# sbarthelemy/arboris-python

Hardware: NVIDIA B200
Metric: world-steps/s (human36, fp64, dt=1ms) (higher is better)
Workload: dtype f64

## Files before the change

arboris-python_b200/csrc/arb_artic.cuh:

```cuda
#pragma once
#include "arb_constraints.cuh"
#include "arb_joints.cuh"
#include "arb_math.cuh"
#include "arb_types.h"

#define FT(ptr, idx) (ptr)[(idx) * ARB_TILE]
#define ST(ptr, idx) (ptr)[(int64_t)(idx) * b.W + w]
ARB_D double arb_ld_state(const double* p) {
#ifdef __CUDA_ARCH__
  double v;
  asm volatile("ld.global.L1::no_allocate.f64 %0, [%1];" : "=d"(v) : "l"(p));
  return v;
#else
  return *p;
#endif
}
#define ST_LD(ptr, idx) arb_ld_state(&ST(ptr, idx))

ARB_HD void wrench_up(const Se3& h, const double* x, double* y) {
  double rm[3], rf[3], c[3];
  m3_mulv(h.R, x, rm);
  m3_mulv(h.R, x + 3, rf);
  cross3(h.p, rf, c);
  y[0] = rm[0] + c[0]; y[1] = rm[1] + c[1]; y[2] = rm[2] + c[2];
// ... 380 lines not shown
#pragma unroll
          for (int i = 0; i < 6; ++i) { IA[6 * r + i] -= U[r] * LA[i]; IM[6 * r + i] -= U[r] * LM[i]; }
          beta[r] += U[r] * u;
        }
      }
    }
    if (par != 0) {
      Se3 X;
      load_se3(b.aX, j, X);
      congruence_up(X, IA);
      congruence_up(X, IM);
      double bu[6];
      wrench_up(X, beta, bu);
      carry = (par == j);
      if (carry) {
#pragma unroll
        for (int i = 0; i < 6; ++i) beta[i] = bu[i];
      } else {
        double* pa = b.aIA + j * (36 * ARB_TILE);
        double* pm = b.aIM + j * (36 * ARB_TILE);
        double* pb = b.abeta + j * (6 * ARB_TILE);
#pragma unroll
        for (int i = 0; i < 36; ++i) { pa[i * ARB_TILE] = IA[i]; pm[i * ARB_TILE] = IM[i]; }
#pragma unroll
        for (int i = 0; i < 6; ++i) pb[i * ARB_TILE] = bu[i];
      }
    } else {
      carry = false;
    }
  }
  return ok;
}

ARB_D bool artic_child_reads_aV(const DevModel& m, int j, int next, bool marked_only) {
  for (int c = m.jchild0[j]; c >= 0; c = m.jsib[c])
    if (c != next && (!marked_only || m.jmark[c])) return true;
  return false;
}
ARB_D bool artic_is_gen_body(const DevModel& m, int j) {
  for (int g = 0; g < m.ngen; ++g)
    if (m.gen_body[g] == j + 1) return true;
  return false;
}
ARB_D int artic_vstride(const DevModel& m) { return 72 * (m.ngen > 1 ? m.ngen : 1); }
ARB_D void artic_down(const Se3& X, double* V, double* Vh) {
  double a[6], c[6];
  iad_apply(X, V, a);
  iad_apply(X, Vh, c);
#pragma unroll
  for (int i = 0; i < 6; ++i) { V[i] = a[i]; Vh[i] = c[i]; }
}

template <bool MARKED_U, int NE, bool PF = true>
ARB_D void artic_forward_full(const DevModel& m, const DevBatch& b, int64_t w, const double* u, double* x,
                              bool ext = false, const int* ek = nullptr) {
  const int n = m.ndof;
  const int VS = artic_vstride(m);
  double V[1 + NE][6], Vh[1 + NE][6];
  int eoff[NE > 0 ? NE : 1], ekc[NE > 0 ? NE : 1];
#pragma unroll
  for (int e = 0; e < NE; ++e) {
    eoff[e] = ext ? m.coloff[m.dofbody[ek[e]]] : 0;
    ekc[e] = ext ? m.dofpos[ek[e]] + 1 : 0;
  }
  int prev = -2;
  for (int j = 0; j < m.nj; ++j) {
    if (PF && j + 1 < m.nj) {
      arb_prefetch_rows<12>(b.aX + (j + 1) * (12 * ARB_TILE));
      artic_prefetch_dofs(m, j + 1, b.aLA, b.aLM, b.aS, b.aSh);
    }
    const int par = m.jparent[j];
    const int nd = arb_joint_ndof(m.jtype[j]);
    const int dof = m.jdof[j];
    const bool ex = NE > 0 && ext && m.jmark[j];
    if (par == 0) {
#pragma unroll
      for (int r = 0; r < 1 + NE; ++r)
#pragma unroll
        for (int i = 0; i < 6; ++i) { V[r][i] = 0.; Vh[r][i] = 0.; }
    } else {
      Se3 X;
      load_se3(b.aX, j, X);
      const bool reload = (par - 1 != prev);
      if (reload) {
#pragma unroll
        for (int i = 0; i < 6; ++i) { V[0][i] = FT(b.aV, (par - 1) * VS + i); Vh[0][i] = FT(b.aV, (par - 1) * VS + 6 + i); }
      }
      artic_down(X, V[0], Vh[0]);
      if (ex) {
#pragma unroll
        for (int e = 1; e < 1 + NE; ++e) {
          if (reload) {
#pragma unroll
            for (int i = 0; i < 6; ++i) {
              V[e][i] = FT(b.aV, (par - 1) * VS + e * 12 + i);
              Vh[e][i] = FT(b.aV, (par - 1) * VS + e * 12 + 6 + i);
            }
          }
          artic_down(X, V[e], Vh[e]);
        }
      }
    }
    const bool useu = !MARKED_U || m.jmark[j];
    for (int c = 0; c < nd; ++c) {
      const int k = dof + c;
      double LA[6], LM[6], s[6], sh[6];
#pragma unroll
      for (int i = 0; i < 6; ++i) {
        LA[i] = FT(b.aLA, k * 6 + i); LM[i] = FT(b.aLM, k * 6 + i);
        s[i] = FT(b.aS, k * 6 + i); sh[i] = FT(b.aSh, k * 6 + i);
      }
      double t = useu ? FT(u, k) : 0.;
      if (par != 0 || c > 0) {
#pragma unroll
        for (int i = 0; i < 6; ++i) t -= LA[i] * V[0][i] + LM[i] * Vh[0][i];
      }
      FT(x, k) = t;
#pragma unroll
      for (int i = 0; i < 6; ++i) { V[0][i] += s[i] * t; Vh[0][i] += sh[i] * t; }
      if (ex) {
        const int pos = m.dofpos[k];
#pragma unroll
        for (int e = 0; e < NE; ++e) {
          const bool onpath = pos < ekc[e] && m.pathdof[eoff[e] + pos] == k;
          double te = onpath ? FT(b.au, (1 + e) * n + k) : 0.;
          if (par != 0 || c > 0) {
#pragma unroll
            for (int i = 0; i < 6; ++i) te -= LA[i] * V[1 + e][i] + LM[i] * Vh[1 + e][i];
          }
          FT(b.ax, e * n + k) = te;
#pragma unroll
          for (int i = 0; i < 6; ++i) { V[1 + e][i] += s[i] * te; Vh[1 + e][i] += sh[i] * te; }
        }
      }
    }
    const bool gen = !MARKED_U && m.jmark[j] && artic_is_gen_body(m, j);
    if (gen || artic_child_reads_aV(m, j, j + 1, false)) {
#pragma unroll
      for (int i = 0; i < 6; ++i) { FT(b.aV, j * VS + i) = V[0][i]; FT(b.aV, j * VS + 6 + i) = Vh[0][i]; }
    }
    if (ex && (gen || artic_child_reads_aV(m, j, j + 1, true))) {
#pragma unroll
      for (int e = 1; e < 1 + NE; ++e)
#pragma unroll
        for (int i = 0; i < 6; ++i) { FT(b.aV, j * VS + e * 12 + i) = V[e][i]; FT(b.aV, j * VS + e * 12 + 6 + i) = Vh[e][i]; }
    }
    prev = j;
  }
}

template <int NR>
ARB_D void artic_backward_generators(const DevModel& m, const DevBatch& b, int64_t w, int body, int kstart,
                                     const double* rot = nullptr, int ubase = 0) {
  const int n = m.ndof;
  const int off = m.coloff[body];
  double beta[NR][6];
#pragma unroll
  for (int r = 0; r < NR; ++r)
#pragma unroll
    for (int i = 0; i < 6; ++i) beta[r][i] = (kstart < 0 && i == r) ? -1. : 0.;
  if (rot != nullptr && NR == 6) {
#pragma unroll
    for (int r = 0; r < NR; ++r)
#pragma unroll
      for (int i = 0; i < 6; ++i) beta[r][i] = ((r < 3) == (i < 3)) ? -rot[3 * (r % 3) + (i % 3)] : 0.;
  }
  const int l0 = (kstart < 0) ? m.kcols[body] - 1 : m.dofpos[kstart];
  for (int l = l0; l >= 0; --l) {
    const int k = m.pathdof[off + l];
    const int j = m.dofjoint[k];
    if (l > 0) {
      const int kn = m.pathdof[off + l - 1];
      arb_prefetch_rows<6>(b.aS + kn * (6 * ARB_TILE));
      arb_prefetch_rows<6>(b.aU + kn * (6 * ARB_TILE));
      arb_prefetch(b.adinv + kn * ARB_TILE);
    }
    double s[6], U[6];
#pragma unroll
    for (int i = 0; i < 6; ++i) { s[i] = FT(b.aS, k * 6 + i); U[i] = FT(b.aU, k * 6 + i); }
    const double dinv = FT(b.adinv, k);
    const bool last = (l == 0);
#pragma unroll
    for (int r = 0; r < NR; ++r) {
      double sb = 0.;
#pragma unroll
      for (int i = 0; i < 6; ++i) sb += s[i] * beta[r][i];
      const double tau = (k == kstart) ? 1. : 0.;
      const double u = (tau - sb) * dinv;
      FT(b.au, (ubase + r) * n + k) = u;
      if (!last) {
#pragma unroll
        for (int i = 0; i < 6; ++i) beta[r][i] += U[i] * u;
      }
    }
    if (k == m.jdof[j] && m.jparent[j] != 0) {
      Se3 X;
      load_se3(b.aX, j, X);
#pragma unroll
      for (int r = 0; r < NR; ++r) {
        double y[6];
        wrench_up(X, beta[r], y);
#pragma unroll
        for (int i = 0; i < 6; ++i) beta[r][i] = y[i];
      }
    }
  }
}

template <int NR, bool CARRY>
ARB_D void artic_forward_generators(const DevModel& m, const DevBatch& b, int64_t w, int body, int kstart) {
  const int n = m.ndof;
  const int VS = artic_vstride(m);
  const int off = m.coloff[body];
  const int kc = ((kstart < 0) ? m.kcols[body] - 1 : m.dofpos[kstart]) + 1;
  double V[NR][6], Vh[NR][6];
  int prev = -2;
  for (int j = 0; j < m.nj; ++j) {
    if (!m.jmark[j]) continue;
    int jn = j + 1;
    while (jn < m.nj && !m.jmark[jn]) ++jn;
    if (jn < m.nj) {
      arb_prefetch_rows<12>(b.aX + jn * (12 * ARB_TILE));
      artic_prefetch_dofs(m, jn, b.aLA, b.aLM, b.aS, b.aSh);
    }
    const int par = m.jparent[j];
    const int nd = arb_joint_ndof(m.jtype[j]);
    const int dof = m.jdof[j];
    if (par == 0) {
#pragma unroll
      for (int r = 0; r < NR; ++r)
#pragma unroll
        for (int i = 0; i < 6; ++i) { V[r][i] = 0.; Vh[r][i] = 0.; }
    } else {
      Se3 X;
      load_se3(b.aX, j, X);
      const bool reload = !CARRY || (par - 1 != prev);
#pragma unroll
      for (int r = 0; r < NR; ++r) {
        if (reload) {
#pragma unroll
          for (int i = 0; i < 6; ++i) {
            V[r][i] = FT(b.aV, (par - 1) * VS + r * 12 + i);
            Vh[r][i] = FT(b.aV, (par - 1) * VS + r * 12 + 6 + i);
          }
        }
        artic_down(X, V[r], Vh[r]);
      }
    }
    for (int c = 0; c < nd; ++c) {
      const int k = dof + c;
      const int pos = m.dofpos[k];
      const bool onpath = pos < kc && m.pathdof[off + pos] == k;
      double LA[6], LM[6], s[6], sh[6];
#pragma unroll
      for (int i = 0; i < 6; ++i) {
        LA[i] = FT(b.aLA, k * 6 + i); LM[i] = FT(b.aLM, k * 6 + i);
        s[i] = FT(b.aS, k * 6 + i); sh[i] = FT(b.aSh, k * 6 + i);
      }
#pragma unroll
      for (int r = 0; r < NR; ++r) {
        double t = onpath ? FT(b.au, r * n + k) : 0.;
        if (par != 0 || c > 0) {
#pragma unroll
          for (int i = 0; i < 6; ++i) t -= LA[i] * V[r][i] + LM[i] * Vh[r][i];
        }
        FT(b.ax, r * n + k) = t;
#pragma unroll
        for (int i = 0; i < 6; ++i) { V[r][i] += s[i] * t; Vh[r][i] += sh[i] * t; }
      }
    }
    if (!CARRY || artic_child_reads_aV(m, j, jn, true)) {
#pragma unroll
      for (int r = 0; r < NR; ++r)
#pragma unroll
        for (int i = 0; i < 6; ++i) {
          FT(b.aV, j * VS + r * 12 + i) = V[r][i];
          FT(b.aV, j * VS + r * 12 + 6 + i) = Vh[r][i];
        }
    } else if (artic_is_gen_body(m, j)) {
#pragma unroll
      for (int r = 0; r < NR; ++r)
#pragma unroll
        for (int i = 0; i < 6; ++i) FT(b.aV, j * VS + r * 12 + i) = V[r][i];
    }
    prev = j;
  }
}

ARB_D void artic_forward_generators_all(const DevModel& m, const DevBatch& b, int64_t w) {
  const int n = m.ndof;
  const int VS = artic_vstride(m);
  for (int j = 0; j < m.nj; ++j) {
    if (!m.jmark[j]) continue;
    int jn = j + 1;
    while (jn < m.nj && !m.jmark[jn]) ++jn;
    if (jn < m.nj) {
      arb_prefetch_rows<12>(b.aX + jn * (12 * ARB_TILE));
      artic_prefetch_dofs(m, jn, b.aLA, b.aLM, b.aS, b.aSh);
    }
    const int par = m.jparent[j];
    const int nd = arb_joint_ndof(m.jtype[j]);
    const int dof = m.jdof[j];
    for (int gi = 0; gi < m.ngen; ++gi) {
      const int off = m.coloff[m.gen_body[gi]];
      const int kc = m.kcols[m.gen_body[gi]];
      const int rb = 6 * gi;
      double V[6][6], Vh[6][6];
      if (par == 0) {
#pragma unroll
        for (int r = 0; r < 6; ++r)
#pragma unroll
          for (int i = 0; i < 6; ++i) { V[r][i] = 0.; Vh[r][i] = 0.; }
      } else {
        Se3 X;
        load_se3(b.aX, j, X);
#pragma unroll
        for (int r = 0; r < 6; ++r) {
#pragma unroll
          for (int i = 0; i < 6; ++i) {
            V[r][i] = FT(b.aV, (par - 1) * VS + (rb + r) * 12 + i);
            Vh[r][i] = FT(b.aV, (par - 1) * VS + (rb + r) * 12 + 6 + i);
          }
          artic_down(X, V[r], Vh[r]);
        }
        if (m.jmarkfirst[j]) {
          const bool pgen = artic_is_gen_body(m, par - 1);
#pragma unroll
          for (int r = 0; r < 6; ++r) {
            const double* pv = b.aV + ((par - 1) * VS + (rb + r) * 12) * ARB_TILE;
            if (!pgen) arb_discard_rows<6>(pv);
            arb_discard_rows<6>(pv + 6 * ARB_TILE);
          }
        }
      }
      for (int c = 0; c < nd; ++c) {
        const int k = dof + c;
        const int pos = m.dofpos[k];
        const bool onpath = pos < kc && m.pathdof[off + pos] == k;
        double LA[6], LM[6], s[6], sh[6];
#pragma unroll
        for (int i = 0; i < 6; ++i) {
          LA[i] = FT(b.aLA, k * 6 + i); LM[i] = FT(b.aLM, k * 6 + i);
          s[i] = FT(b.aS, k * 6 + i); sh[i] = FT(b.aSh, k * 6 + i);
        }
#pragma unroll
        for (int r = 0; r < 6; ++r) {
          double t = onpath ? FT(b.au, (rb + r) * n + k) : 0.;
          if (par != 0 || c > 0) {
#pragma unroll
            for (int i = 0; i < 6; ++i) t -= LA[i] * V[r][i] + LM[i] * Vh[r][i];
          }
          if (m.doflim[k]) FT(b.ax, (rb + r) * n + k) = t;
#pragma unroll
          for (int i = 0; i < 6; ++i) { V[r][i] += s[i] * t; Vh[r][i] += sh[i] * t; }
        }
      }
      const bool vh_read = m.jmarkchild[j] != 0;
#pragma unroll
      for (int r = 0; r < 6; ++r)
#pragma unroll
        for (int i = 0; i < 6; ++i) {
          FT(b.aV, j * VS + (rb + r) * 12 + i) = V[r][i];
          if (vh_read) FT(b.aV, j * VS + (rb + r) * 12 + 6 + i) = Vh[r][i];
        }
    }
  }
}

#ifndef ARTIC_GEN_CARRY
#define ARTIC_GEN_CARRY 0
#endif
template <int NR>
ARB_D void artic_solve_generators(const DevModel& m, const DevBatch& b, int64_t w, int body, int kstart,
                                  const double* rot = nullptr) {
  artic_backward_generators<NR>(m, b, w, body, kstart, rot, 0);
  artic_forward_generators<NR, (ARTIC_GEN_CARRY != 0)>(m, b, w, body, kstart);
}

ARB_D double artic_gen_value(const DevModel& m, const DevBatch& b, int64_t w, int g, int r, const double* x) {
  if (g < 6 * m.ngen) return FT(b.aV, (m.gen_body[g / 6] - 1) * artic_vstride(m) + r * 12 + g % 6);
  return FT(x, r * m.ndof + m.glimdof[g - 6 * m.ngen]);
}
ARB_D void artic_gen_block(const DevModel& m, const DevBatch& b, int gi, int r, const double* rot, double* out) {
  double V[6];
#pragma unroll
  for (int i = 0; i < 6; ++i) V[i] = FT(b.aV, (m.gen_body[gi] - 1) * artic_vstride(m) + r * 12 + i);
  if (rot != nullptr) {
    m3_mulv(rot, V, out);
    m3_mulv(rot, V + 3, out + 3);
  } else {
#pragma unroll
    for (int i = 0; i < 6; ++i) out[i] = V[i];
  }
}

ARB_D void artic_backward_wrenches(const DevModel& m, const DevBatch& b, int64_t w, const double* y) {
  const int NG6 = 6 * m.ngen;
  for (int j = m.nj - 1; j >= 0; --j) {
    if (!m.jmark[j]) continue;
    const int par = m.jparent[j];
    const int nd = arb_joint_ndof(m.jtype[j]);
    const int dof = m.jdof[j];
    double beta[6] = {0., 0., 0., 0., 0., 0.};
    for (int g = 0; g < m.ngen; ++g)
      if (m.gen_body[g] == j + 1) {
        if (m.gen_aligned[g]) {
          double Re[9], yy[6], t[6];
#pragma unroll
          for (int i = 0; i < 9; ++i) Re[i] = FT(b.fRe, 9 * g + i);
#pragma unroll
          for (int i = 0; i < 6; ++i) yy[i] = FT(y, 6 * g + i);
          m3t_mulv(Re, yy, t);
          m3t_mulv(Re, yy + 3, t + 3);
#pragma unroll
          for (int i = 0; i < 6; ++i) beta[i] -= t[i];
        } else {
#pragma unroll
          for (int i = 0; i < 6; ++i) beta[i] -= FT(y, 6 * g + i);
        }
// ... 32 lines not shown
```

arboris-python_b200/csrc/arb_fused.cuh:

```cuda
#pragma once
#include "arb_artic.cuh"
#include "arb_constraints.cuh"
#include "arb_world.cuh"

ARB_D DevBatch fused_tile_view(const DevBatch& b, int64_t w) {
  DevBatch t = b;
  const int64_t tile = w / ARB_TILE, lane = w % ARB_TILE;
  const int64_t od = tile * b.frec * ARB_TILE + lane, oi = tile * b.firec * ARB_TILE + lane;
  t.fq += od; t.fLam += od; t.fv0 += od; t.fT1 += od; t.fT0 += od; t.fu += od; t.fy += od;
  t.fAcc += od; t.fP += od; t.faux += od; t.fpose += od; t.ff += od; t.fRe += od;
  t.aX += od; t.atw += od; t.ath += od; t.aS += od; t.aSh += od; t.aU += od; t.aLA += od;
  t.aLM += od; t.adinv += od; t.aIA += od; t.aIM += od; t.abeta += od; t.au += od; t.ax += od;
  t.aV += od; t.fK += od;
  t.factive += oi; t.fbranch += oi; t.fzidx += oi;
  return t;
}

ARB_D bool constraint_update(const DevModel& m, int c, const Se3& P0, const Se3& P1, const double* TW0,
                             const double* TW1, double q, double dt, double* aux, double* T1,
                             double* T0, int* zidx, bool aligned = false) {
  const int type = m.ctype[c];
  const double* cd = m.cdbl + ARB_CONS_NDBL * c;
  if (type == ARB_CONS_JOINT_LIMITS) {
    aux[0] = q;
// ... 28 lines not shown
    aux[0] = sdist;
    r0 = 2; nr = 4;
    if (!active) return false;
    if (aligned) {
      const double d[3] = {P1.p[0] - Hc0.p[0], P1.p[1] - Hc0.p[1], P1.p[2] - Hc0.p[2]};
      m3t_mulv(Hc0.R, d, T1);
      return true;
    }
  }
  Se3 F0, F1, F0i, H01;
  se3_mul(P0, cb0, F0);
  se3_mul(P1, cb1, F1);
  se3_inv(F0, F0i);
  se3_mul(F0i, F1, H01);
  if (type == ARB_CONS_BALL_SOCKET) {
#pragma unroll
    for (int i = 0; i < 3; ++i) aux[i] = H01.p[i];
  }
#pragma unroll
  for (int col = 0; col < 6; ++col) {
    double e[6] = {0., 0., 0., 0., 0., 0.}, y[6], z[6];
    e[col] = 1.;
    iad_apply(cb1, e, y);
    ad_apply(H01, y, z);
    for (int r = 0; r < nr; ++r) T1[r * 6 + col] = z[r0 + r];
    iad_apply(cb0, e, y);
    for (int r = 0; r < nr; ++r) T0[r * 6 + col] = y[r0 + r];
  }
  return true;
}

template <int NR>
ARB_D void fused_gen_rows(const DevModel& m, const DevBatch& b, int64_t w, const double* x, double* out,
                          int stride, int col0, int rv0 = 0) {
  for (int gj = 0; gj < m.ngen; ++gj) {
    double Re[9];
    const bool al = m.gen_aligned[gj] != 0;
    if (al) {
#pragma unroll
      for (int i = 0; i < 9; ++i) Re[i] = FT(b.fRe, 9 * gj + i);
    }
#pragma unroll
    for (int r = 0; r < NR; ++r) {
      double v[6];
      artic_gen_block(m, b, gj, rv0 + r, al ? Re : nullptr, v);
#pragma unroll
      for (int i = 0; i < 6; ++i) FT(out, (6 * gj + i) * stride + col0 + r) = v[i];
    }
  }
  for (int g = 6 * m.ngen; g < m.ngrows; ++g)
#pragma unroll
    for (int r = 0; r < NR; ++r) FT(out, g * stride + col0 + r) = FT(x, r * m.ndof + m.glimdof[g - 6 * m.ngen]);
}

template <bool APPLIED = false>
ARB_D void world_fused_prepare(const DevModel& m, const DevBatch& b, int64_t w, double dt,
                               const DevApplied& ap = DevApplied{nullptr, nullptr, nullptr}) {
  const int NG = m.ngrows;
  artic_kinematics(m, b, w);
  if (!artic_factor<APPLIED>(m, b, w, dt, ap)) b.status[w] |= ARB_STATUS_SINGULAR;
  for (int gi = 0; gi < m.ngen; ++gi) {
    if (!m.gen_aligned[gi]) continue;
    double Rc[9], Rb[9], Re[9];
    int zi[3];
    zaligned(m.cdbl + ARB_CONS_NDBL * m.gen_c0[gi] + 32, Rc, zi);
#pragma unroll
    for (int i = 0; i < 9; ++i) Rb[i] = FT(b.fpose, (m.gen_body[gi] - 1) * 12 + i);
#pragma unroll
    for (int i = 0; i < 3; ++i)
#pragma unroll
      for (int j = 0; j < 3; ++j) Re[3 * i + j] = Rc[i] * Rb[j] + Rc[3 + i] * Rb[3 + j] + Rc[6 + i] * Rb[6 + j];
#pragma unroll
    for (int i = 0; i < 9; ++i) FT(b.fRe, 9 * gi + i) = Re[i];
  }
  bool any = false;
  for (int c = 0; c < m.nc; ++c) {
    const int* ci = m.cint + ARB_CONS_NINT * c;
    const int type = m.ctype[c];
// ... 12 lines not shown
    } else {
      Se3 P0, P1;
      double TW0[6], TW1[6];
      if (ci[0] == 0) se3_identity(P0); else load_se3(b.fpose, ci[0] - 1, P0);
      if (ci[1] == 0) se3_identity(P1); else load_se3(b.fpose, ci[1] - 1, P1);
#pragma unroll
      for (int i = 0; i < 6; ++i) {
        TW0[i] = (ci[0] == 0) ? 0. : FT(b.atw, (ci[0] - 1) * 6 + i);
        TW1[i] = (ci[1] == 0) ? 0. : FT(b.atw, (ci[1] - 1) * 6 + i);
      }
      const bool aligned = m.caligned[c] != 0;
      act = constraint_update(m, c, P0, P1, TW0, TW1, 0., dt, aux, T1, T0, zi, aligned);
      if (type == ARB_CONS_SOFT_FINGER_PLANE_POINT) {
#pragma unroll
        for (int i = 0; i < 4; ++i) ST(b.cforce, r0 + i) = 0.;
#pragma unroll
        for (int i = 0; i < 3; ++i) FT(b.fzidx, 3 * c + i) = zi[i];
      }
      if (act) {
        if (aligned) {
#pragma unroll
          for (int i = 0; i < 3; ++i) FT(b.fT1, c * 24 + i) = T1[i];
        } else {
          const int nr = arb_cons_ndol(type);
          for (int i = 0; i < nr * 6; ++i) { FT(b.fT1, c * 24 + i) = T1[i]; FT(b.fT0, c * 24 + i) = T0[i]; }
        }
      }
    }
#pragma unroll
    for (int i = 0; i < 4; ++i) FT(b.faux, 4 * c + i) = aux[i];
    FT(b.factive, c) = act ? 1 : 0;
    any = any || act;
  }
  const int nlim = NG - 6 * m.ngen;
  const int nm = nlim >= 2 ? 2 : 0;
  if (nm == 2) {
    const int ek[2] = {m.glimdof[0], m.glimdof[1]};
    if (any) {
      artic_backward_generators<1>(m, b, w, m.dofbody[ek[0]], ek[0], nullptr, 1);
      artic_backward_generators<1>(m, b, w, m.dofbody[ek[1]], ek[1], nullptr, 2);
    }
    artic_forward_full<false, 2>(m, b, w, b.au, b.fq, any, ek);
  } else {
    artic_forward_full<false, 0>(m, b, w, b.au, b.fq);
  }
  if (!any) return;
  fused_gen_rows<1>(m, b, w, b.fq, b.fv0, 1, 0);
  for (int e = 0; e < nm; ++e)
    fused_gen_rows<1>(m, b, w, b.ax + e * m.ndof * ARB_TILE, b.fLam, NG, 6 * m.ngen + e, 1 + e);
#ifndef PREP_GEN_SEPARATE
  for (int gi = 0; gi < m.ngen; ++gi) {
    if (m.gen_aligned[gi]) {
      double Re[9];
#pragma unroll
      for (int i = 0; i < 9; ++i) Re[i] = FT(b.fRe, 9 * gi + i);
      artic_backward_generators<6>(m, b, w, m.gen_body[gi], -1, Re, 6 * gi);
    } else {
      artic_backward_generators<6>(m, b, w, m.gen_body[gi], -1, nullptr, 6 * gi);
    }
  }
  artic_forward_generators_all(m, b, w);
  for (int gi = 0; gi < m.ngen; ++gi)
    fused_gen_rows<6>(m, b, w, b.ax + 6 * gi * m.ndof * ARB_TILE, b.fLam, NG, 6 * gi, 6 * gi);
#else
  for (int gi = 0; gi < m.ngen; ++gi) {
    if (m.gen_aligned[gi]) {
      double Re[9];
#pragma unroll
      for (int i = 0; i < 9; ++i) Re[i] = FT(b.fRe, 9 * gi + i);
      artic_solve_generators<6>(m, b, w, m.gen_body[gi], -1, Re);
    } else {
      artic_solve_generators<6>(m, b, w, m.gen_body[gi], -1);
    }
    fused_gen_rows<6>(m, b, w, b.ax, b.fLam, NG, 6 * gi);
  }
#endif
  for (int h = 6 * m.ngen + nm; h < NG; ++h) {
    const int k = m.glimdof[h - 6 * m.ngen];
    artic_solve_generators<1>(m, b, w, m.dofbody[k], k);
    fused_gen_rows<1>(m, b, w, b.ax, b.fLam, NG, h);
  }
}

#ifdef __CUDA_ARCH__
#define arb_warp_any(pred) (__any_sync(__activemask(), (pred)) != 0)
#else
#define arb_warp_any(pred) (pred)
#endif

ARB_D void gs_prefetch_visit(const DevModel& m, const DevBatch& b, int c) {
  const int r0 = m.crow[c];
  const double* Tp = ((m.cgen1[c] < 0) ? b.fT0 : b.fT1) + c * (24 * ARB_TILE);
  const double* pA = b.fAcc + r0 * (4 * ARB_TILE);
  const double* pP = b.fP + r0 * (4 * ARB_TILE);
  if (m.caligned[c]) {
#pragma unroll
    for (int i = 0; i < 3; ++i) arb_prefetch(Tp + i * ARB_TILE);
  } else {
#pragma unroll
    for (int i = 0; i < 24; ++i) arb_prefetch(Tp + i * ARB_TILE);
  }
#pragma unroll
  for (int i = 0; i < 16; ++i) { arb_prefetch(pA + i * ARB_TILE); arb_prefetch(pP + i * ARB_TILE); }
}

struct GsCache {
  int g, n;
  double u[6], dy[6];
  double* L;
  int ls;
};
#define GSL(k, i) (k).L[(i) * (k).ls]

ARB_D void gs_cache_flush(const DevModel& m, const DevBatch& b, int64_t w, GsCache& k) {
// ... 1200 lines not shown
      if (needs && k.g != gF) {
        gs_cache_flush(m, b, w, k);
        gs_cache_load<true>(m, b, w, k, gF, 6);
      }
      if (type == ARB_CONS_BALL_SOCKET) {
        if (act) gs_visit_one_body<3>(m, b, w, c, dt, k, &status);
        continue;
      }
      double f[4], df[4];
      int br = 0, slot = 0;
      if (act) {
        if (c + 1 < m.nc) gs_prefetch_visit(m, b, c + 1);
        br = gs_softfinger_begin(m, b, c, dt, k, co, f, df, &slot, &status);
      }
      coop_solve_sliding(co, m.cdbl + ARB_CONS_NDBL * c + 37);
      if (act) gs_softfinger_end(m, b, c, k, co, br, slot, f, df, &status);
      if (br == 3 && c < 32) slid |= 1u << c;
    }
  }
  if (live) {
    gs_cache_flush(m, b, w, k);
    gs_final_wrench(m, b);
    for (int r = 0; r < m.nrows; ++r) ST(b.cforce, r) = FT(b.ff, r);
    if (status) b.status[w] |= status;
  }
  return gs_sort_key(m, slid, (unsigned)(amask & 0xffffffffull));
}

ARB_D void world_fused_finish(const DevModel& m, const DevBatch& b, int64_t w, double dt) {
  bool any = false;
  for (int c = 0; c < m.nc; ++c) any = any || FT(b.factive, c);
  if (any) {
    artic_backward_wrenches(m, b, w, b.fy);
    artic_forward_full<true, 0, false>(m, b, w, b.au, b.ax);
  }
  bool finite = true;
  for (int j = 0; j < m.nj; ++j) {
    const int type = m.jtype[j];
    const int g = m.jgpos[j], d = m.jdof[j];
    const int nd = arb_joint_ndof(type);
    double nv[6];
    for (int i = 0; i < nd; ++i) {
      double t = FT(b.fq, d + i);
      if (any) t += FT(b.ax, d + i);
      ST(b.gvel, d + i) = t;
      finite = finite && isfinite(t);
      nv[i] = t;
    }
    if (type == ARB_JOINT_FREE) {
      double q[16], tw[6];
      for (int i = 0; i < 16; ++i) q[i] = ST_LD(b.gpos, g + i);
#pragma unroll
      for (int i = 0; i < 6; ++i) tw[i] = dt * nv[i];
      Se3 H, E, R;
      se3_from16(q, H);
      se3_exp(tw, E);
      se3_mul(H, E, R);
#pragma unroll
      for (int r = 0; r < 3; ++r) {
#pragma unroll
        for (int c = 0; c < 3; ++c) ST(b.gpos, g + 4 * r + c) = R.R[3 * r + c];
        ST(b.gpos, g + 4 * r + 3) = R.p[r];
      }
    } else {
      for (int i = 0; i < nd; ++i) ST(b.gpos, g + i) = ST_LD(b.gpos, g + i) + dt * nv[i];
    }
  }
// ... 3 lines not shown
```

arboris-python_b200/csrc/arb_model_host.h:

```cpp
#pragma once
#include <cmath>
#include <cstring>
#include <string>
#include <vector>
#include "arb_math.cuh"
#include "arb_types.h"

struct HostModel {
  int ndof = 0, ngpos = 0, nj = 0, nc = 0, na = 0, nrows = 0, ncols = 0, maxk = 0, anyvisc = 0;
  std::vector<int> jtype, jparent, jdof, jgpos, hcn_ident, bflags, coloff, kcols, pathdof;
  std::vector<int> ctype, cint, crow, atype, aint;
  std::vector<int> dofbody, dofpos, gen_body, cgen1, cgen0;
  std::vector<int> gen_aligned, gen_c0, caligned;
  std::vector<int> doflim;
  std::vector<unsigned> crunmask;
  int ngen = 0, ngrows = 0;
  std::vector<int> dofjoint, jhaschild, jaccfirst, jmark, jmarkfirst, jmarkchild, glimdof, pd_gpos;
  std::vector<int> pd_index, pd_dofs;
  int has_warm = 0;
  std::vector<int> glev_off, glev_joint, gslot, gvslot;
  GroupLayout gl;
  std::vector<int> jchild0, jsib;
  std::vector<double> pd_kp, pd_kd, pd_qd, pd_c, pd_dqd;
  int has_pd = 0, nweight = 0;
// ... 315 lines not shown
  }
  int64_t total_ints() const { return cactive + cbranch + cdol + czidx; }
};
static inline ScratchSizes scratch_sizes(const HostModel& m) {
  ScratchSizes s;
  const int64_t n = m.ndof, nj = m.nj, nr = m.nrows > 0 ? m.nrows : 1, nc = m.nc > 0 ? m.nc : 1;
  s.pose = nj * 12; s.twist = nj * 6; s.J = (int64_t)m.ncols * 6; s.dJ = s.J;
  s.M = s.N = s.B = s.Z = s.Y = n * n; s.gforce = n;
  s.cjac = nr * n; s.cvel = nr; s.cA = nr * nr; s.cT = n * nr; s.cpinv = nr * 4; s.caux = nc * 4;
  s.tmp = 2 * n;
  s.cactive = s.cbranch = s.cdol = nc; s.czidx = nc * 3;
  return s;
}
struct FusedSizes {
  int64_t fq, fLam, fv0, fT1, fT0, fu, fy, fAcc, fP, faux, fpose, ff, fRe, factive, fbranch, fzidx;
  int64_t aX, atw, ath, aS, aSh, aU, aLA, aLM, adinv, aIA, aIM, abeta, au, ax, aV, fK;
  int64_t total_doubles() const {
    return fq + fLam + fv0 + fT1 + fT0 + fu + fy + fAcc + fP + faux + fpose + ff + fRe +
           aX + atw + ath + aS + aSh + aU + aLA + aLM + adinv + aIA + aIM + abeta + au + ax + aV + fK;
  }
  int64_t total_ints() const { return factive + fbranch + fzidx; }
};
static inline FusedSizes fused_sizes(const HostModel& m) {
  FusedSizes s;
  const int64_t n = m.ndof, NG = m.ngrows > 0 ? m.ngrows : 1, nc = m.nc > 0 ? m.nc : 1,
                nr = m.nrows > 0 ? m.nrows : 1;
  const int64_t nj = m.nj > 0 ? m.nj : 1, nn = n > 0 ? n : 1;
  s.fq = nn; s.fLam = NG * NG; s.fv0 = NG; s.fT1 = nc * 24; s.fT0 = nc * 24;
  s.fu = NG; s.fy = NG; s.fAcc = nr * 4; s.fP = nr * 4; s.faux = nc * 4; s.fpose = nj * 12; s.ff = nr;
  s.fRe = 9 * (m.ngen > 0 ? m.ngen : 1);
  s.factive = nc; s.fbranch = nc; s.fzidx = 3 * nc;
  s.aX = nj * 12; s.atw = nj * 6; s.ath = nj * 6;
  s.aS = s.aSh = s.aU = s.aLA = s.aLM = nn * 6; s.adinv = nn;
  s.aIA = s.aIM = nj * 36; s.abeta = nj * 6;
  const int64_t ng1 = m.ngen > 1 ? m.ngen : 1;
  s.au = 6 * ng1 * nn; s.ax = 6 * ng1 * nn; s.aV = nj * 72 * ng1;
  s.fK = nn * NG;
  return s;
}
static inline int64_t fused_padded_worlds(int64_t W) { return (W + ARB_TILE - 1) / ARB_TILE * ARB_TILE; }
static inline void carve_fused(const FusedSizes& s, double* dbl, int* ints, DevBatch& b) {
  double* p = dbl;
  auto take = [&](int64_t k) { double* r = p; p += k * ARB_TILE; return r; };
  b.fq = take(s.fq); b.fLam = take(s.fLam); b.fv0 = take(s.fv0);
  b.fT1 = take(s.fT1); b.fT0 = take(s.fT0); b.fu = take(s.fu); b.fy = take(s.fy);
  b.fAcc = take(s.fAcc); b.fP = take(s.fP); b.faux = take(s.faux); b.fpose = take(s.fpose);
  b.ff = take(s.ff); b.fRe = take(s.fRe);
  b.aX = take(s.aX); b.atw = take(s.atw); b.ath = take(s.ath);
  b.aS = take(s.aS); b.aSh = take(s.aSh); b.aU = take(s.aU); b.aLA = take(s.aLA); b.aLM = take(s.aLM);
  b.adinv = take(s.adinv); b.aIA = take(s.aIA); b.aIM = take(s.aIM); b.abeta = take(s.abeta);
  b.au = take(s.au); b.ax = take(s.ax); b.aV = take(s.aV);
  b.fK = take(s.fK);
  int* q = ints;
  auto takei = [&](int64_t k) { int* r = q; q += k * ARB_TILE; return r; };
  b.factive = takei(s.factive); b.fbranch = takei(s.fbranch); b.fzidx = takei(s.fzidx);
  b.frec = s.total_doubles();
  b.firec = s.total_ints();
}
static inline int applied_wrench_rows(const HostModel& m, int nbodies, const int32_t* bodies, bool has_wrench,
                                      std::vector<int>& rows, std::string& err) {
  if (nbodies < 0) { err = "negative number of wrench bodies"; return -1; }
  if (nbodies > 0 && !bodies) { err = "null body list"; return -1; }
  if (has_wrench && nbodies == 0) { err = "a wrench array needs its bodies"; return -1; }
  rows.assign(m.nj > 0 ? m.nj : 1, -1);
  for (int i = 0; i < nbodies; ++i) {
    const int body = bodies[i];
    if (body == 0) { err = "no wrench can be applied to the ground (body 0)"; return -1; }
    if (body < 0 || body > m.nj) { err = "wrench body " + std::to_string(body) + " out of range"; return -1; }
    if (rows[body - 1] >= 0) { err = "wrench body " + std::to_string(body) + " listed twice"; return -1; }
// ... 18 lines not shown
```

Before: 23.54 million.

## Fuse all generator backward/forward sweeps into single per-joint tree passes

Replaces the separate backward and forward articulated-body sweeps, previously run once per generator group (6-row body generators and single-row joint-limit rows), with one backward pass over marked joints that handles every group per joint. Generator columns are also folded into the main forward_full sweep per joint. Partial beta wrenches are carried across joints in an abeta slot buffer, and the aV/au/ax buffers are resized to hold all NG rows. The aim is fewer traversals of the tree and reuse of per-joint S/U/LA/LM loads across groups, at the cost of larger per-world scratch buffers and more global memory traffic for the carried state.

After: 21.86 million, median of 6. 0.929x the previous value.

```diff
diff --git a/arboris-python_b200/csrc/arb_artic.cuh b/arboris-python_b200/csrc/arb_artic.cuh
--- a/arboris-python_b200/csrc/arb_artic.cuh
+++ b/arboris-python_b200/csrc/arb_artic.cuh
@@ -436,6 +436,16 @@
   return ok;
 }
 
+ARB_D int artic_vstride(const DevModel& m) { return 12 * (1 + m.ngrows); }
+
+#ifdef ARB_HOSTTEST_COUNTERS
+#define ARB_ROWREADS_MAXJ 256
+static long arb_rowreads[2][ARB_ROWREADS_MAXJ];
+#define ARB_COUNT_ROWS(dir, j) do { if ((j) < ARB_ROWREADS_MAXJ) ++arb_rowreads[dir][j]; } while (0)
+#else
+#define ARB_COUNT_ROWS(dir, j) do { } while (0)
+#endif
+
 ARB_D bool artic_child_reads_aV(const DevModel& m, int j, int next, bool marked_only) {
   for (int c = m.jchild0[j]; c >= 0; c = m.jsib[c])
     if (c != next && (!marked_only || m.jmark[c])) return true;
@@ -446,7 +456,6 @@
     if (m.gen_body[g] == j + 1) return true;
   return false;
 }
-ARB_D int artic_vstride(const DevModel& m) { return 72 * (m.ngen > 1 ? m.ngen : 1); }
 ARB_D void artic_down(const Se3& X, double* V, double* Vh) {
   double a[6], c[6];
   iad_apply(X, V, a);
@@ -455,20 +464,83 @@
   for (int i = 0; i < 6; ++i) { V[i] = a[i]; Vh[i] = c[i]; }
 }
 
-template <bool MARKED_U, int NE, bool PF = true>
-ARB_D void artic_forward_full(const DevModel& m, const DevBatch& b, int64_t w, const double* u, double* x,
-                              bool ext = false, const int* ek = nullptr) {
+template <int NR>
+ARB_D void artic_forward_group(const DevModel& m, const DevBatch& b, int j, int g0, int off, int kc) {
   const int n = m.ndof;
   const int VS = artic_vstride(m);
-  double V[1 + NE][6], Vh[1 + NE][6];
-  int eoff[NE > 0 ? NE : 1], ekc[NE > 0 ? NE : 1];
-#pragma unroll
-  for (int e = 0; e < NE; ++e) {
-    eoff[e] = ext ? m.coloff[m.dofbody[ek[e]]] : 0;
-    ekc[e] = ext ? m.dofpos[ek[e]] + 1 : 0;
-  }
+  const int cv = 1 + g0;
+  const int par = m.jparent[j];
+  const int nd = arb_joint_ndof(m.jtype[j]);
+  const int dof = m.jdof[j];
+  double V[NR][6], Vh[NR][6];
+  if (par == 0) {
+#pragma unroll
+    for (int r = 0; r < NR; ++r)
+#pragma unroll
+      for (int i = 0; i < 6; ++i) { V[r][i] = 0.; Vh[r][i] = 0.; }
+  } else {
+    Se3 X;
+    load_se3(b.aX, j, X);
+#pragma unroll
+    for (int r = 0; r < NR; ++r) {
+#pragma unroll
+      for (int i = 0; i < 6; ++i) {
+        V[r][i] = FT(b.aV, (par - 1) * VS + (cv + r) * 12 + i);
+        Vh[r][i] = FT(b.aV, (par - 1) * VS + (cv + r) * 12 + 6 + i);
+      }
+      artic_down(X, V[r], Vh[r]);
+    }
+    if (m.jmarkfirst[j]) {
+      const bool pgen = artic_is_gen_body(m, par - 1);
+#pragma unroll
+      for (int r = 0; r < NR; ++r) {
+        const double* pv = b.aV + ((par - 1) * VS + (cv + r) * 12) * ARB_TILE;
+        if (!pgen) arb_discard_rows<6>(pv);
+        arb_discard_rows<6>(pv + 6 * ARB_TILE);
+      }
+    }
+  }
+  for (int c = 0; c < nd; ++c) {
+    const int k = dof + c;
+    const int pos = m.dofpos[k];
+    const bool onpath = pos < kc && m.pathdof[off + pos] == k;
+    double LA[6], LM[6], s[6], sh[6];
+#pragma unroll
+    for (int i = 0; i < 6; ++i) {
+      LA[i] = FT(b.aLA, k * 6 + i); LM[i] = FT(b.aLM, k * 6 + i);
+      s[i] = FT(b.aS, k * 6 + i); sh[i] = FT(b.aSh, k * 6 + i);
+    }
+#pragma unroll
+    for (int r = 0; r < NR; ++r) {
+      double t = onpath ? FT(b.au, (cv + r) * n + k) : 0.;
+      if (par != 0 || c > 0) {
+#pragma unroll
+        for (int i = 0; i < 6; ++i) t -= LA[i] * V[r][i] + LM[i] * Vh[r][i];
+      }
+      if (m.doflim[k]) FT(b.ax, (g0 + r) * n + k) = t;
+#pragma unroll
+      for (int i = 0; i < 6; ++i) { V[r][i] += s[i] * t; Vh[r][i] += sh[i] * t; }
+    }
+  }
+  const bool vh_read = m.jmarkchild[j] != 0;
+#pragma unroll
+  for (int r = 0; r < NR; ++r)
+#pragma unroll
+    for (int i = 0; i < 6; ++i) {
+      FT(b.aV, j * VS + (cv + r) * 12 + i) = V[r][i];
+      if (vh_read) FT(b.aV, j * VS + (cv + r) * 12 + 6 + i) = Vh[r][i];
+    }
+}
+
+template <bool MARKED_U, bool GEN, bool PF = true>
+ARB_D void artic_forward_full(const DevModel& m, const DevBatch& b, int64_t w, const double* u, double* x,
+                              bool gens = false) {
+  const int VS = artic_vstride(m);
+  const int NG6 = 6 * m.ngen;
+  double V[6], Vh[6];
   int prev = -2;
   for (int j = 0; j < m.nj; ++j) {
+    ARB_COUNT_ROWS(1, j);
     if (PF && j + 1 < m.nj) {
       arb_prefetch_rows<12>(b.aX + (j + 1) * (12 * ARB_TILE));
       artic_prefetch_dofs(m, j + 1, b.aLA, b.aLM, b.aS, b.aSh);
@@ -476,34 +548,17 @@
     const int par = m.jparent[j];
     const int nd = arb_joint_ndof(m.jtype[j]);
     const int dof = m.jdof[j];
-    const bool ex = NE > 0 && ext && m.jmark[j];
     if (par == 0) {
 #pragma unroll
-      for (int r = 0; r < 1 + NE; ++r)
-#pragma unroll
-        for (int i = 0; i < 6; ++i) { V[r][i] = 0.; Vh[r][i] = 0.; }
+      for (int i = 0; i < 6; ++i) { V[i] = 0.; Vh[i] = 0.; }
     } else {
       Se3 X;
       load_se3(b.aX, j, X);
-      const bool reload = (par - 1 != prev);
-      if (reload) {
-#pragma unroll
-        for (int i = 0; i < 6; ++i) { V[0][i] = FT(b.aV, (par - 1) * VS + i); Vh[0][i] = FT(b.aV, (par - 1) * VS + 6 + i); }
-      }
-      artic_down(X, V[0], Vh[0]);
-      if (ex) {
-#pragma unroll
-        for (int e = 1; e < 1 + NE; ++e) {
-          if (reload) {
-#pragma unroll
-            for (int i = 0; i < 6; ++i) {
-              V[e][i] = FT(b.aV, (par - 1) * VS + e * 12 + i);
-              Vh[e][i] = FT(b.aV, (par - 1) * VS + e * 12 + 6 + i);
-            }
-          }
-          artic_down(X, V[e], Vh[e]);
-        }
-      }
+      if (par - 1 != prev) {
+#pragma unroll
+        for (int i = 0; i < 6; ++i) { V[i] = FT(b.aV, (par - 1) * VS + i); Vh[i] = FT(b.aV, (par - 1) * VS + 6 + i); }
+      }
+      artic_down(X, V, Vh);
     }
     const bool useu = !MARKED_U || m.jmark[j];
     for (int c = 0; c < nd; ++c) {
@@ -517,68 +572,60 @@
       double t = useu ? FT(u, k) : 0.;
       if (par != 0 || c > 0) {
 #pragma unroll
-        for (int i = 0; i < 6; ++i) t -= LA[i] * V[0][i] + LM[i] * Vh[0][i];
+        for (int i = 0; i < 6; ++i) t -= LA[i] * V[i] + LM[i] * Vh[i];
       }
       FT(x, k) = t;
 #pragma unroll
-      for (int i = 0; i < 6; ++i) { V[0][i] += s[i] * t; Vh[0][i] += sh[i] * t; }
-      if (ex) {
-        const int pos = m.dofpos[k];
-#pragma unroll
-        for (int e = 0; e < NE; ++e) {
-          const bool onpath = pos < ekc[e] && m.pathdof[eoff[e] + pos] == k;
-          double te = onpath ? FT(b.au, (1 + e) * n + k) : 0.;
-          if (par != 0 || c > 0) {
-#pragma unroll
-            for (int i = 0; i < 6; ++i) te -= LA[i] * V[1 + e][i] + LM[i] * Vh[1 + e][i];
-          }
-          FT(b.ax, e * n + k) = te;
-#pragma unroll
-          for (int i = 0; i < 6; ++i) { V[1 + e][i] += s[i] * te; Vh[1 + e][i] += sh[i] * te; }
-        }
-      }
+      for (int i = 0; i < 6; ++i) { V[i] += s[i] * t; Vh[i] += sh[i] * t; }
     }
     const bool gen = !MARKED_U && m.jmark[j] && artic_is_gen_body(m, j);
     if (gen || artic_child_reads_aV(m, j, j + 1, false)) {
 #pragma unroll
-      for (int i = 0; i < 6; ++i) { FT(b.aV, j * VS + i) = V[0][i]; FT(b.aV, j * VS + 6 + i) = Vh[0][i]; }
-    }
-    if (ex && (gen || artic_child_reads_aV(m, j, j + 1, true))) {
-#pragma unroll
-      for (int e = 1; e < 1 + NE; ++e)
-#pragma unroll
-        for (int i = 0; i < 6; ++i) { FT(b.aV, j * VS + e * 12 + i) = V[e][i]; FT(b.aV, j * VS + e * 12 + 6 + i) = Vh[e][i]; }
+      for (int i = 0; i < 6; ++i) { FT(b.aV, j * VS + i) = V[i]; FT(b.aV, j * VS + 6 + i) = Vh[i]; }
     }
     prev = j;
+    if (GEN && gens && m.jmark[j]) {
+      for (int gi = 0; gi < m.ngen; ++gi)
+        artic_forward_group<6>(m, b, j, 6 * gi, m.coloff[m.gen_body[gi]], m.kcols[m.gen_body[gi]]);
+      for (int g = NG6; g < m.ngrows; ++g) {
+        const int k = m.glimdof[g - NG6];
+        artic_forward_group<1>(m, b, j, g, m.coloff[m.dofbody[k]], m.dofpos[k] + 1);
+      }
+    }
   }
 }
 
 template <int NR>
-ARB_D void artic_backward_generators(const DevModel& m, const DevBatch& b, int64_t w, int body, int kstart,
-                                     const double* rot = nullptr, int ubase = 0) {
+ARB_D void artic_backward_group(const DevModel& m, const DevBatch& b, int j, int g0, int body, int kstart, int rot) {
   const int n = m.ndof;
-  const int off = m.coloff[body];
+  const int dof = m.jdof[j];
+  const int p0 = m.dofpos[dof];
+  const int l0 = (kstart < 0) ? m.kcols[body] - 1 : m.dofpos[kstart];
+  if (p0 > l0 || m.pathdof[m.coloff[body] + p0] != dof) return;
+  double* slot = b.abeta + g0 * (6 * ARB_TILE);
   double beta[NR][6];
-#pragma unroll
-  for (int r = 0; r < NR; ++r)
-#pragma unroll
-    for (int i = 0; i < 6; ++i) beta[r][i] = (kstart < 0 && i == r) ? -1. : 0.;
-  if (rot != nullptr && NR == 6) {
+  if (j == body - 1) {
 #pragma unroll
     for (int r = 0; r < NR; ++r)
 #pragma unroll
-      for (int i = 0; i < 6; ++i) beta[r][i] = ((r < 3) == (i < 3)) ? -rot[3 * (r % 3) + (i % 3)] : 0.;
-  }
-  const int l0 = (kstart < 0) ? m.kcols[body] - 1 : m.dofpos[kstart];
-  for (int l = l0; l >= 0; --l) {
-    const int k = m.pathdof[off + l];
-    const int j = m.dofjoint[k];
-    if (l > 0) {
-      const int kn = m.pathdof[off + l - 1];
-      arb_prefetch_rows<6>(b.aS + kn * (6 * ARB_TILE));
-      arb_prefetch_rows<6>(b.aU + kn * (6 * ARB_TILE));
-      arb_prefetch(b.adinv + kn * ARB_TILE);
-    }
+      for (int i = 0; i < 6; ++i) beta[r][i] = (kstart < 0 && i == r) ? -1. : 0.;
+    if (rot >= 0 && NR == 6) {
+      const double* R = b.fRe + 9 * rot * ARB_TILE;
+#pragma unroll
+      for (int r = 0; r < NR; ++r)
+#pragma unroll
+        for (int i = 0; i < 6; ++i) beta[r][i] = ((r < 3) == (i < 3)) ? -FT(R, 3 * (r % 3) + (i % 3)) : 0.;
+    }
+  } else {
+#pragma unroll
+    for (int r = 0; r < NR; ++r)
+#pragma unroll
+      for (int i = 0; i < 6; ++i) beta[r][i] = FT(slot, 6 * r + i);
+  }
+  for (int c = arb_joint_ndof(m.jtype[j]) - 1; c >= 0; --c) {
+    const int l = p0 + c;
+    if (l > l0) continue;
+    const int k = dof + c;
     double s[6], U[6];
 #pragma unroll
     for (int i = 0; i < 6; ++i) { s[i] = FT(b.aS, k * 6 + i); U[i] = FT(b.aU, k * 6 + i); }
@@ -591,204 +638,58 @@
       for (int i = 0; i < 6; ++i) sb += s[i] * beta[r][i];
       const double tau = (k == kstart) ? 1. : 0.;
       const double u = (tau - sb) * dinv;
-      FT(b.au, (ubase + r) * n + k) = u;
+      FT(b.au, (1 + g0 + r) * n + k) = u;
       if (!last) {
 #pragma unroll
         for (int i = 0; i < 6; ++i) beta[r][i] += U[i] * u;
       }
     }
-    if (k == m.jdof[j] && m.jparent[j] != 0) {
-      Se3 X;
-      load_se3(b.aX, j, X);
-#pragma unroll
-      for (int r = 0; r < NR; ++r) {
-        double y[6];
-        wrench_up(X, beta[r], y);
-#pragma unroll
-        for (int i = 0; i < 6; ++i) beta[r][i] = y[i];
-      }
-    }
-  }
-}
-
-template <int NR, bool CARRY>
-ARB_D void artic_forward_generators(const DevModel& m, const DevBatch& b, int64_t w, int body, int kstart) {
-  const int n = m.ndof;
-  const int VS = artic_vstride(m);
-  const int off = m.coloff[body];
-  const int kc = ((kstart < 0) ? m.kcols[body] - 1 : m.dofpos[kstart]) + 1;
-  double V[NR][6], Vh[NR][6];
-  int prev = -2;
-  for (int j = 0; j < m.nj; ++j) {
+  }
+  if (m.jparent[j] != 0) {
+    Se3 X;
+    load_se3(b.aX, j, X);
+#pragma unroll
+    for (int r = 0; r < NR; ++r) {
+      double y[6];
+      wrench_up(X, beta[r], y);
+#pragma unroll
+      for (int i = 0; i < 6; ++i) FT(slot, 6 * r + i) = y[i];
+    }
+  } else {
+    arb_discard_rows<6 * NR>(slot);
+  }
+}
+
+ARB_D void artic_backward_generators(const DevModel& m, const DevBatch& b, int64_t w) {
+  const int NG6 = 6 * m.ngen;
+  for (int j = m.nj - 1; j >= 0; --j) {
     if (!m.jmark[j]) continue;
-    int jn = j + 1;
-    while (jn < m.nj && !m.jmark[jn]) ++jn;
-    if (jn < m.nj) {
-      arb_prefetch_rows<12>(b.aX + jn * (12 * ARB_TILE));
-      artic_prefetch_dofs(m, jn, b.aLA, b.aLM, b.aS, b.aSh);
-    }
-    const int par = m.jparent[j];
-    const int nd = arb_joint_ndof(m.jtype[j]);
-    const int dof = m.jdof[j];
-    if (par == 0) {
-#pragma unroll
-      for (int r = 0; r < NR; ++r)
-#pragma unroll
-        for (int i = 0; i < 6; ++i) { V[r][i] = 0.; Vh[r][i] = 0.; }
-    } else {
-      Se3 X;
-      load_se3(b.aX, j, X);
-      const bool reload = !CARRY || (par - 1 != prev);
-#pragma unroll
-      for (int r = 0; r < NR; ++r) {
-        if (reload) {
-#pragma unroll
-          for (int i = 0; i < 6; ++i) {
-            V[r][i] = FT(b.aV, (par - 1) * VS + r * 12 + i);
-            Vh[r][i] = FT(b.aV, (par - 1) * VS + r * 12 + 6 + i);
-          }
-        }
-        artic_down(X, V[r], Vh[r]);
-      }
-    }
-    for (int c = 0; c < nd; ++c) {
-      const int k = dof + c;
-      const int pos = m.dofpos[k];
-      const bool onpath = pos < kc && m.pathdof[off + pos] == k;
-      double LA[6], LM[6], s[6], sh[6];
-#pragma unroll
-      for (int i = 0; i < 6; ++i) {
-        LA[i] = FT(b.aLA, k * 6 + i); LM[i] = FT(b.aLM, k * 6 + i);
-        s[i] = FT(b.aS, k * 6 + i); sh[i] = FT(b.aSh, k * 6 + i);
-      }
-#pragma unroll
-      for (int r = 0; r < NR; ++r) {
-        double t = onpath ? FT(b.au, r * n + k) : 0.;
-        if (par != 0 || c > 0) {
-#pragma unroll
-          for (int i = 0; i < 6; ++i) t -= LA[i] * V[r][i] + LM[i] * Vh[r][i];
-        }
-        FT(b.ax, r * n + k) = t;
-#pragma unroll
-        for (int i = 0; i < 6; ++i) { V[r][i] += s[i] * t; Vh[r][i] += sh[i] * t; }
-      }
-    }
-    if (!CARRY || artic_child_reads_aV(m, j, jn, true)) {
-#pragma unroll
-      for (int r = 0; r < NR; ++r)
-#pragma unroll
-        for (int i = 0; i < 6; ++i) {
-          FT(b.aV, j * VS + r * 12 + i) = V[r][i];
-          FT(b.aV, j * VS + r * 12 + 6 + i) = Vh[r][i];
-        }
-    } else if (artic_is_gen_body(m, j)) {
-#pragma unroll
-      for (int r = 0; r < NR; ++r)
-#pragma unroll
-        for (int i = 0; i < 6; ++i) FT(b.aV, j * VS + r * 12 + i) = V[r][i];
-    }
-    prev = j;
-  }
-}
-
-ARB_D void artic_forward_generators_all(const DevModel& m, const DevBatch& b, int64_t w) {
-  const int n = m.ndof;
-  const int VS = artic_vstride(m);
-  for (int j = 0; j < m.nj; ++j) {
-    if (!m.jmark[j]) continue;
-    int jn = j + 1;
-    while (jn < m.nj && !m.jmark[jn]) ++jn;
-    if (jn < m.nj) {
-      arb_prefetch_rows<12>(b.aX + jn * (12 * ARB_TILE));
-      artic_prefetch_dofs(m, jn, b.aLA, b.aLM, b.aS, b.aSh);
-    }
-    const int par = m.jparent[j];
-    const int nd = arb_joint_ndof(m.jtype[j]);
-    const int dof = m.jdof[j];
-    for (int gi = 0; gi < m.ngen; ++gi) {
-      const int off = m.coloff[m.gen_body[gi]];
-      const int kc = m.kcols[m.gen_body[gi]];
-      const int rb = 6 * gi;
-      double V[6][6], Vh[6][6];
-      if (par == 0) {
-#pragma unroll
-        for (int r = 0; r < 6; ++r)
-#pragma unroll
-          for (int i = 0; i < 6; ++i) { V[r][i] = 0.; Vh[r][i] = 0.; }
-      } else {
-        Se3 X;
-        load_se3(b.aX, j, X);
-#pragma unroll
-        for (int r = 0; r < 6; ++r) {
-#pragma unroll
-          for (int i = 0; i < 6; ++i) {
-            V[r][i] = FT(b.aV, (par - 1) * VS + (rb + r) * 12 + i);
-            Vh[r][i] = FT(b.aV, (par - 1) * VS + (rb + r) * 12 + 6 + i);
-          }
-          artic_down(X, V[r], Vh[r]);
-        }
-        if (m.jmarkfirst[j]) {
-          const bool pgen = artic_is_gen_body(m, par - 1);
-#pragma unroll
-          for (int r = 0; r < 6; ++r) {
-            const double* pv = b.aV + ((par - 1) * VS + (rb + r) * 12) * ARB_TILE;
-            if (!pgen) arb_discard_rows<6>(pv);
-            arb_discard_rows<6>(pv + 6 * ARB_TILE);
-          }
-        }
-      }
+    ARB_COUNT_ROWS(0, j);
+    int jn = j - 1;
+    while (jn >= 0 && !m.jmark[jn]) --jn;
+    if (jn >= 0) {
+      if (m.jparent[jn] != 0) arb_prefetch_rows<12>(b.aX + jn * (12 * ARB_TILE));
+      const int nd = arb_joint_ndof(m.jtype[jn]);
       for (int c = 0; c < nd; ++c) {
-        const int k = dof + c;
-        const int pos = m.dofpos[k];
-        const bool onpath = pos < kc && m.pathdof[off + pos] == k;
-        double LA[6], LM[6], s[6], sh[6];
-#pragma unroll
-        for (int i = 0; i < 6; ++i) {
-          LA[i] = FT(b.aLA, k * 6 + i); LM[i] = FT(b.aLM, k * 6 + i);
-          s[i] = FT(b.aS, k * 6 + i); sh[i] = FT(b.aSh, k * 6 + i);
-        }
-#pragma unroll
-        for (int r = 0; r < 6; ++r) {
-          double t = onpath ? FT(b.au, (rb + r) * n + k) : 0.;
-          if (par != 0 || c > 0) {
-#pragma unroll
-            for (int i = 0; i < 6; ++i) t -= LA[i] * V[r][i] + LM[i] * Vh[r][i];
-          }
-          if (m.doflim[k]) FT(b.ax, (rb + r) * n + k) = t;
-#pragma unroll
-          for (int i = 0; i < 6; ++i) { V[r][i] += s[i] * t; Vh[r][i] += sh[i] * t; }
-        }
-      }
-      const bool vh_read = m.jmarkchild[j] != 0;
-#pragma unroll
-      for (int r = 0; r < 6; ++r)
-#pragma unroll
-        for (int i = 0; i < 6; ++i) {
-          FT(b.aV, j * VS + (rb + r) * 12 + i) = V[r][i];
-          if (vh_read) FT(b.aV, j * VS + (rb + r) * 12 + 6 + i) = Vh[r][i];
-        }
-    }
-  }
-}
-
-#ifndef ARTIC_GEN_CARRY
-#define ARTIC_GEN_CARRY 0
-#endif
-template <int NR>
-ARB_D void artic_solve_generators(const DevModel& m, const DevBatch& b, int64_t w, int body, int kstart,
-                                  const double* rot = nullptr) {
-  artic_backward_generators<NR>(m, b, w, body, kstart, rot, 0);
-  artic_forward_generators<NR, (ARTIC_GEN_CARRY != 0)>(m, b, w, body, kstart);
-}
-
-ARB_D double artic_gen_value(const DevModel& m, const DevBatch& b, int64_t w, int g, int r, const double* x) {
-  if (g < 6 * m.ngen) return FT(b.aV, (m.gen_body[g / 6] - 1) * artic_vstride(m) + r * 12 + g % 6);
-  return FT(x, r * m.ndof + m.glimdof[g - 6 * m.ngen]);
-}
-ARB_D void artic_gen_block(const DevModel& m, const DevBatch& b, int gi, int r, const double* rot, double* out) {
+        const int kn = m.jdof[jn] + c;
+        arb_prefetch_rows<6>(b.aS + kn * (6 * ARB_TILE));
+        arb_prefetch_rows<6>(b.aU + kn * (6 * ARB_TILE));
+        arb_prefetch(b.adinv + kn * ARB_TILE);
+      }
+    }
+    for (int gi = 0; gi < m.ngen; ++gi)
+      artic_backward_group<6>(m, b, j, 6 * gi, m.gen_body[gi], -1, m.gen_aligned[gi] ? gi : -1);
+    for (int g = NG6; g < m.ngrows; ++g) {
+      const int k = m.glimdof[g - NG6];
+      artic_backward_group<1>(m, b, j, g, m.dofbody[k], k, -1);
+    }
+  }
+}
+
+ARB_D void artic_gen_block(const DevModel& m, const DevBatch& b, int gi, int cv, const double* rot, double* out) {
   double V[6];
 #pragma unroll
-  for (int i = 0; i < 6; ++i) V[i] = FT(b.aV, (m.gen_body[gi] - 1) * artic_vstride(m) + r * 12 + i);
+  for (int i = 0; i < 6; ++i) V[i] = FT(b.aV, (m.gen_body[gi] - 1) * artic_vstride(m) + cv * 12 + i);
   if (rot != nullptr) {
     m3_mulv(rot, V, out);
     m3_mulv(rot, V + 3, out + 3);
diff --git a/arboris-python_b200/csrc/arb_fused.cuh b/arboris-python_b200/csrc/arb_fused.cuh
--- a/arboris-python_b200/csrc/arb_fused.cuh
+++ b/arboris-python_b200/csrc/arb_fused.cuh
@@ -84,7 +84,7 @@
 
 template <int NR>
 ARB_D void fused_gen_rows(const DevModel& m, const DevBatch& b, int64_t w, const double* x, double* out,
-                          int stride, int col0, int rv0 = 0) {
+                          int stride, int col0, int cv0) {
   for (int gj = 0; gj < m.ngen; ++gj) {
     double Re[9];
     const bool al = m.gen_aligned[gj] != 0;
@@ -95,7 +95,7 @@
 #pragma unroll
     for (int r = 0; r < NR; ++r) {
       double v[6];
-      artic_gen_block(m, b, gj, rv0 + r, al ? Re : nullptr, v);
+      artic_gen_block(m, b, gj, cv0 + r, al ? Re : nullptr, v);
 #pragma unroll
       for (int i = 0; i < 6; ++i) FT(out, (6 * gj + i) * stride + col0 + r) = v[i];
     }
@@ -174,54 +174,14 @@
     FT(b.factive, c) = act ? 1 : 0;
     any = any || act;
   }
-  const int nlim = NG - 6 * m.ngen;
-  const int nm = nlim >= 2 ? 2 : 0;
-  if (nm == 2) {
-    const int ek[2] = {m.glimdof[0], m.glimdof[1]};
-    if (any) {
-      artic_backward_generators<1>(m, b, w, m.dofbody[ek[0]], ek[0], nullptr, 1);
-      artic_backward_generators<1>(m, b, w, m.dofbody[ek[1]], ek[1], nullptr, 2);
-    }
-    artic_forward_full<false, 2>(m, b, w, b.au, b.fq, any, ek);
-  } else {
-    artic_forward_full<false, 0>(m, b, w, b.au, b.fq);
-  }
+  if (any) artic_backward_generators(m, b, w);
+  artic_forward_full<false, true>(m, b, w, b.au, b.fq, any);
   if (!any) return;
-  fused_gen_rows<1>(m, b, w, b.fq, b.fv0, 1, 0);
-  for (int e = 0; e < nm; ++e)
-    fused_gen_rows<1>(m, b, w, b.ax + e * m.ndof * ARB_TILE, b.fLam, NG, 6 * m.ngen + e, 1 + e);
-#ifndef PREP_GEN_SEPARATE
-  for (int gi = 0; gi < m.ngen; ++gi) {
-    if (m.gen_aligned[gi]) {
-      double Re[9];
-#pragma unroll
-      for (int i = 0; i < 9; ++i) Re[i] = FT(b.fRe, 9 * gi + i);
-      artic_backward_generators<6>(m, b, w, m.gen_body[gi], -1, Re, 6 * gi);
-    } else {
-      artic_backward_generators<6>(m, b, w, m.gen_body[gi], -1, nullptr, 6 * gi);
-    }
-  }
-  artic_forward_generators_all(m, b, w);
+  fused_gen_rows<1>(m, b, w, b.fq, b.fv0, 1, 0, 0);
   for (int gi = 0; gi < m.ngen; ++gi)
-    fused_gen_rows<6>(m, b, w, b.ax + 6 * gi * m.ndof * ARB_TILE, b.fLam, NG, 6 * gi, 6 * gi);
-#else
-  for (int gi = 0; gi < m.ngen; ++gi) {
-    if (m.gen_aligned[gi]) {
-      double Re[9];
-#pragma unroll
-      for (int i = 0; i < 9; ++i) Re[i] = FT(b.fRe, 9 * gi + i);
-      artic_solve_generators<6>(m, b, w, m.gen_body[gi], -1, Re);
-    } else {
-      artic_solve_generators<6>(m, b, w, m.gen_body[gi], -1);
-    }
-    fused_gen_rows<6>(m, b, w, b.ax, b.fLam, NG, 6 * gi);
-  }
-#endif
-  for (int h = 6 * m.ngen + nm; h < NG; ++h) {
-    const int k = m.glimdof[h - 6 * m.ngen];
-    artic_solve_generators<1>(m, b, w, m.dofbody[k], k);
-    fused_gen_rows<1>(m, b, w, b.ax, b.fLam, NG, h);
-  }
+    fused_gen_rows<6>(m, b, w, b.ax + 6 * gi * m.ndof * ARB_TILE, b.fLam, NG, 6 * gi, 1 + 6 * gi);
+  for (int g = 6 * m.ngen; g < NG; ++g)
+    fused_gen_rows<1>(m, b, w, b.ax + g * m.ndof * ARB_TILE, b.fLam, NG, g, 1 + g);
 }
 
 #ifdef __CUDA_ARCH__
@@ -1488,7 +1448,7 @@
   for (int c = 0; c < m.nc; ++c) any = any || FT(b.factive, c);
   if (any) {
     artic_backward_wrenches(m, b, w, b.fy);
-    artic_forward_full<true, 0, false>(m, b, w, b.au, b.ax);
+    artic_forward_full<true, false, false>(m, b, w, b.au, b.ax);
   }
   bool finite = true;
   for (int j = 0; j < m.nj; ++j) {
diff --git a/arboris-python_b200/csrc/arb_model_host.h b/arboris-python_b200/csrc/arb_model_host.h
--- a/arboris-python_b200/csrc/arb_model_host.h
+++ b/arboris-python_b200/csrc/arb_model_host.h
@@ -371,9 +371,8 @@
   s.factive = nc; s.fbranch = nc; s.fzidx = 3 * nc;
   s.aX = nj * 12; s.atw = nj * 6; s.ath = nj * 6;
   s.aS = s.aSh = s.aU = s.aLA = s.aLM = nn * 6; s.adinv = nn;
-  s.aIA = s.aIM = nj * 36; s.abeta = nj * 6;
-  const int64_t ng1 = m.ngen > 1 ? m.ngen : 1;
-  s.au = 6 * ng1 * nn; s.ax = 6 * ng1 * nn; s.aV = nj * 72 * ng1;
+  s.aIA = s.aIM = nj * 36; s.abeta = (nj > NG ? nj : NG) * 6;
+  s.au = (1 + NG) * nn; s.ax = NG * nn; s.aV = nj * 12 * (1 + NG);
   s.fK = nn * NG;
   return s;
 }
```
